# calderpg/fast_kinematic_simulator

Measured on AMD Instinct MI355X. Metric: particle-microsteps/sec, 7-DOF arm vs 256³ SDF, at 1/2/4/8 MI355X, higher is better.
Workload: dtype f64

## Files before the change

### fast_kinematic_simulator_amd/_capi.py

```python
from __future__ import annotations

import ctypes
import os
from ctypes import POINTER, c_char_p, c_double, c_float, c_int32, c_int64, c_uint8, c_uint32, c_uint64, c_void_p

LIB_NAME = "libfks_hip.so"
LIB_PATH = os.environ.get("FKS_LIB_PATH") or os.path.join(os.path.dirname(os.path.abspath(__file__)), LIB_NAME)

FKS_OK = 0
STATUS_NAMES = {
    0: "FKS_OK",
    1: "FKS_ERR_INVALID_ARGUMENT",
    2: "FKS_ERR_HIP",
    3: "FKS_ERR_NO_ROBOT",
    4: "FKS_ERR_OUT_OF_MEMORY",
    5: "FKS_ERR_UNSUPPORTED",
    6: "FKS_ERR_NO_DEVICE",
}

ROBOT_LINKED, ROBOT_SE2, ROBOT_SE3 = 0, 1, 2
JOINT_FIXED, JOINT_REVOLUTE, JOINT_CONTINUOUS, JOINT_PRISMATIC = 0, 1, 2, 4
KIN_LINK_TRANSFORMS, KIN_POINTS, KIN_APPLY_CONTROL_INPUT = 0, 1, 2
OK, ERR_INVALID_ARGUMENT, ERR_HIP, ERR_NO_ROBOT, ERR_OUT_OF_MEMORY, ERR_UNSUPPORTED, ERR_NO_DEVICE = 0, 1, 2, 3, 4, 5, 6

NUM_PHASES = 16
PHASE_NAMES = ["particle", "control", "step_setup", "micro_input", "micro_fk", "env_check", "self_check", "corrections",
               "solve", "resolve_apply", "output", "env_rounds_skipped", "env_rounds_evaluated", "corr_rounds_skipped",
               "corr_rounds_evaluated", "wave_residency"]
PHASE_COUNTS = {"env_rounds_skipped", "env_rounds_evaluated", "corr_rounds_skipped", "corr_rounds_evaluated", "wave_residency"}

PARTICLE_ERR_MICROSTEP_MOTION = 0x1
PARTICLE_ERR_NORMAL_OOB = 0x2
PARTICLE_ERR_ZERO_DIRECTION = 0x4
PARTICLE_ERR_RNG_EXHAUSTED = 0x8
PARTICLE_ERR_SELF_CAPACITY = 0x10
PARTICLE_ERR_KEY_RANGE = 0x20
PARTICLE_ERR_MICROSTEP_CAP = 0x40
PARTICLE_ERR_SELF_SINGULAR = 0x80
PARTICLE_ERR_NO_NOISE_BIN = 0x100


class SolverParams(ctypes.Structure):
    _fields_ = [
        ("forward_simulation_time", c_double),
        ("simulation_shortcut_distance", c_double),
        ("environment_collision_check_tolerance", c_double),
        ("resolve_correction_step_scaling_decay_rate", c_double),
        ("resolve_correction_initial_step_size", c_double),
        ("resolve_correction_min_step_scaling", c_double),
        ("max_resolver_iterations", c_uint32),
        ("resolve_correction_step_scaling_decay_iterations", c_uint32),
        ("failed_resolves_end_motion", c_uint32),
        ("reserved", c_uint32),
    ]


class GridGeometry(ctypes.Structure):
    _fields_ = [("origin", c_double * 12), ("resolution", c_double), ("num_cells", c_int64 * 3)]


class Environment(ctypes.Structure):
    _fields_ = [
        ("collision_map", GridGeometry),
        ("sdf", GridGeometry),
        ("sdf_values", POINTER(c_float)),
        ("sdf_oob_value", c_float),
        ("reserved", c_uint32),
        ("normals", GridGeometry),
        ("normal_offsets", POINTER(c_uint32)),
        ("normal_entries", POINTER(c_double)),
    ]


class DofController(ctypes.Structure):
    _fields_ = [
        ("kp", c_double),
        ("ki", c_double),
        ("kd", c_double),
        ("integral_clamp", c_double),
        ("velocity_limit", c_double),
        ("acceleration_limit", c_double),
        ("max_sensor_noise", c_double),
        ("max_actuator_proportional_noise", c_double),
        ("max_actuator_minimum_noise", c_double),
    ]


class JointDesc(ctypes.Structure):
    _fields_ = [
        ("parent_link", c_int32),
        ("child_link", c_int32),
        ("type", c_int32),
        ("reserved", c_int32),
        ("origin", c_double * 12),
        ("axis", c_double * 3),
        ("limit_lower", c_double),
        ("limit_upper", c_double),
    ]


class SampledActuator(ctypes.Structure):
    _fields_ = [
        ("num_bins", c_uint32),
        ("bin_elements", c_uint32),
        ("bin_bounds", POINTER(c_double)),
        ("bin_samples", POINTER(c_double)),
    ]


class RobotDesc(ctypes.Structure):
    _fields_ = [
        ("robot_type", c_int32),
# ... 354 lines not shown
```

### fast_kinematic_simulator_amd/csrc/fks_kernels.hip

```cpp
#if !defined(__HIPCC_RTC__)
#include <hip/hip_runtime.h>
#include <stdint.h>
#endif

#include "fks_capi.h"
#include "fks_control.h"
#include "fks_device.h"
#include "fks_portable_math.h"
#include "fks_se3.h"

namespace fksd {

using fks_math::clamp;
using fks_math::dabs;
using fks_math::dmax;
using fks_math::dmin;
using fks_math::dsqrt;

#if defined(FKS_SHAPE_L)
struct RobotShape {
    int L, J, D, W, G;
};
constexpr RobotShape kShape{FKS_SHAPE_L, FKS_SHAPE_J, FKS_SHAPE_D, FKS_SHAPE_W, FKS_SHAPE_G};
constexpr LdsLayout kShapeLayout = make_lds_layout(FKS_SHAPE_L, FKS_SHAPE_J, FKS_SHAPE_D, FKS_SHAPE_W, FKS_SHAPE_G,
// ... 233 lines not shown
        c[3] = lo0;
        k0 += W0;
        k1 += W1;
    }
}
__device__ __forceinline__ double u53(uint32_t a, uint32_t b) {
    const uint64_t bits = (((uint64_t)a << 32) | (uint64_t)b) >> 11;
    return (double)bits * (1.0 / 9007199254740992.0);
}
__device__ double tn_sample(uint32_t k0, uint32_t k1, uint64_t particle, uint32_t step, uint32_t micro, uint32_t dof,
                            uint32_t* err) {
    const double mean = 0.0, stddev = 0.5, lo = -2.0, hi = 2.0;
    uint32_t attempt = 0;
    while (attempt < 64u) {
        double x, y, r2;
        for (;;) {
            uint32_t c[4] = {(uint32_t)particle, step, micro,
                             ((uint32_t)(particle >> 32) << 16) | ((dof & 0xffu) << 8) | attempt};
            philox4x32_10(c, k0, k1);
            x = 2.0 * u53(c[0], c[1]) - 1.0;
            y = 2.0 * u53(c[2], c[3]) - 1.0;
            r2 = x * x + y * y;
            if (!(r2 > 1.0 || r2 == 0.0)) break;
            if (++attempt >= 64u) {
                *err |= FKS_PARTICLE_ERR_RNG_EXHAUSTED;
                return 0.0;
            }
        }
        const double mult = dsqrt(-2.0 * fks_math::log(r2) / r2);
        const double n1 = (y * mult) * 1.0 + 0.0;
        const double n2 = (x * mult) * 1.0 + 0.0;
        if ((n1 <= hi) && (n1 >= lo)) return mean + stddev * n1;
        if ((n2 <= hi) && (n2 >= lo)) return mean + stddev * n2;
        ++attempt;
    }
    *err |= FKS_PARTICLE_ERR_RNG_EXHAUSTED;
    return 0.0;
}

__device__ double sampled_pick(uint32_t k0, uint32_t k1, uint64_t particle, uint32_t step, uint32_t micro, uint32_t dof,
                               uint32_t elems) {
    uint32_t c[4] = {(uint32_t)particle, step, micro, ((uint32_t)(particle >> 32) << 16) | ((dof & 0xffu) << 8)};
    philox4x32_10(c, k0, k1);
    uint32_t pick = (uint32_t)(u53(c[0], c[1]) * (double)elems);
    if (pick >= elems) pick = elems - 1u;
    return (double)pick;
}

struct Sim;
__device__ FKS_SHAPE_INLINE void refill_noise(Sim& s, uint32_t micro0, uint32_t M);
__device__ __forceinline__ double noise_sample(Sim& s, uint32_t micro);

__device__ __forceinline__ bool grid_index(const GridDev& g, const D4& p, int32_t idx[3]) {
    const D4 q = xform4(g.inv, p);
    const double v[3] = {q.x * g.inv_res, q.y * g.inv_res, q.z * g.inv_res};
    bool ok = true;
#pragma unroll
    for (int a = 0; a < 3; ++a) {
        const bool fin = (v[a] > -2147483648.0) && (v[a] < 2147483647.0);
        idx[a] = fin ? (int32_t)v[a] : -1;
        ok = ok && fin && idx[a] >= 0 && (int64_t)idx[a] < g.n[a];
    }
    return ok;
}
__device__ __forceinline__ uint32_t grid_brick(const GridDev& g, int32_t i, int32_t j, int32_t k) {
    return brick_cell(g.nb, (uint32_t)i, (uint32_t)j, (uint32_t)k);
}

#ifndef FKS_ASM_LANE
#if defined(FKS_SHAPE_LEAN) && FKS_SHAPE_LEAN
#define FKS_ASM_LANE 1
#else
#define FKS_ASM_LANE 0
#endif
#endif
#if defined(FKS_SHAPE_TYPE) && FKS_SHAPE_TYPE == 0
#define FKS_PID_REGS 0
#else
#define FKS_PID_REGS 1
#endif
#ifndef FKS_PAR_PROOF
#define FKS_PAR_PROOF 1
#endif
#ifndef FKS_NO_SKIP_PROOFS
#define FKS_NO_SKIP_PROOFS 0
#endif
extern __shared__ __attribute__((aligned(16))) double fks_lds[];

struct Sim {
    const SimArgs* A;
    double* lds_block;
    double* scratch;
    int lane_v;
    __device__ __forceinline__ int lane() const {
#if FKS_ASM_LANE
        int ln;
        asm volatile("v_mbcnt_lo_u32_b32 %0, -1, 0\n\tv_mbcnt_hi_u32_b32 %0, -1, %0" : "=v"(ln));
        return ln;
#else
        return lane_v;
#endif
    }
    uint32_t step;
    uint32_t err;
    uint64_t lane_bytes;
    uint64_t local;
    uint32_t micro_count, resolver_count, step_count, lsq_rows;
    __device__ __forceinline__ double* lds() const { return lds_block; }
    __device__ __forceinline__ double* shared() const { return fks_lds; }
    __device__ __forceinline__ uint64_t pid() const { return A->first_pid + local; }
    __device__ __forceinline__ uint32_t* stats() const { return reinterpret_cast<uint32_t*>(lds() + LAY(*A).misc + 24); }
    __device__ __forceinline__ uint64_t* phase() const { return reinterpret_cast<uint64_t*>(lds() + LAY(*A).misc + 8); }
    __device__ __forceinline__ uint64_t* totals() const { return reinterpret_cast<uint64_t*>(lds() + LAY(*A).misc + 32); }
    __device__ __forceinline__ const JointDev* joints() const { return reinterpret_cast<const JointDev*>(shared() + LAY(*A).joints); }
    __device__ __forceinline__ const fks_dof_controller* ctrl() const {
        return reinterpret_cast<const fks_dof_controller*>(shared() + LAY(*A).ctrl);
    }
    __device__ __forceinline__ const int32_t* dofj() const { return reinterpret_cast<const int32_t*>(shared() + LAY(*A).dofj); }
    __device__ __forceinline__ const double* base() const { return shared() + LAY(*A).base; }
    __device__ __forceinline__ double* pid_state() const { return scratch + SLAY(*A).pid; }
#if FKS_PID_REGS
    double pid_integral, pid_last;
#endif
    double* rstate;
    double* selfref;
    bool self_nonempty;
    bool tcur_valid;
    uint32_t tr_steps, tr_cfgs;
};
template <int RT>
__device__ __forceinline__ void pid_get(const Sim& s, int ln, double* integral, double* last) {
    if constexpr (RT == FKS_ROBOT_LINKED) {
        *integral = s.pid_state()[ln];
        *last = s.pid_state()[kWave + ln];
    } else {
#if FKS_PID_REGS
        *integral = s.pid_integral;
        *last = s.pid_last;
#endif
    }
}
template <int RT>
__device__ __forceinline__ void pid_set(Sim& s, int ln, double integral, double last) {
    if constexpr (RT == FKS_ROBOT_LINKED) {
        s.pid_state()[ln] = integral;
        s.pid_state()[kWave + ln] = last;
    } else {
#if FKS_PID_REGS
        s.pid_integral = integral;
        s.pid_last = last;
#endif
    }
}
enum { kTotSteps = 0, kTotMicro, kTotResolver, kTotLsq, kTotErrors, kWaveTotals };

__device__ __forceinline__ int opaque_lane(int ln) {
    asm volatile("" : "+v"(ln));
    return ln;
}

__device__ __forceinline__ uint64_t* self_counters(const Sim& s) { return reinterpret_cast<uint64_t*>(s.lds() + LAY(*s.A).misc + 28); }

template <bool TR>
__device__ __forceinline__ void trace_config(Sim& s, const double* cfg, uint32_t micro, uint32_t kind) {
    if constexpr (TR) {
        const SimArgs& A = *s.A;
        const uint32_t k = s.tr_cfgs++;
        if (k < A.tr_cfg_cap) {
            const uint64_t rec = s.local * (uint64_t)A.tr_cfg_cap + k;
            if (s.lane() < RDIM(A.R, W)) A.tr_cfg[rec * (uint64_t)RDIM(A.R, W) + s.lane()] = cfg[s.lane()];
            if (s.lane() == 0) {
                A.tr_tags[3 * rec] = s.step;
                A.tr_tags[3 * rec + 1] = micro;
                A.tr_tags[3 * rec + 2] = kind;
            }
        }
    }
}
template <bool TR>
__device__ __forceinline__ void trace_step(Sim& s, const double* u, const double* ustep, uint32_t M) {
    if constexpr (TR) {
        const SimArgs& A = *s.A;
        const uint32_t k = s.tr_steps++;
        if (k < A.tr_step_cap) {
            const int D = RDIM(A.R, D);
            const uint64_t rec = s.local * (uint64_t)A.tr_step_cap + k;
            if (s.lane() < D) {
                A.tr_inputs[rec * 2ull * (uint64_t)D + s.lane()] = u[s.lane()];
                A.tr_inputs[rec * 2ull * (uint64_t)D + D + s.lane()] = ustep[s.lane()];
            }
            if (s.lane() == 0) A.tr_micro[rec] = M;
        }
    }
}

#ifndef FKS_PHASE_TIMERS
#define FKS_PHASE_TIMERS 0
#endif
__device__ __forceinline__ uint64_t tick() {
    if constexpr (FKS_PHASE_TIMERS) return __builtin_amdgcn_s_memtime();
    return 0;
}
__device__ __forceinline__ void tock(Sim& s, int phase, uint64_t t0) {
    if constexpr (FKS_PHASE_TIMERS)
        if (s.lane() == 0) s.phase()[phase] += tick() - t0;
}
__device__ __forceinline__ void count_event(Sim& s, int slot, uint64_t n) {
    if constexpr (FKS_PHASE_TIMERS)
        if (s.lane() == 0) s.phase()[slot] += n;
}

__device__ __noinline__ void refill_noise_lanes(const SimArgs* __restrict__ Ap, double* lds, int ln, uint64_t pid, uint32_t step,
                                                uint32_t micro0, uint32_t M) {
    const SimArgs& A = *Ap;
    const int D = RDIM(A.R, D);
    const int per = kWave / D;
    double* nz = lds + LAY(A).noise;
    uint32_t* ne = reinterpret_cast<uint32_t*>(lds + LAY(A).noise_err);
    if (ln < per * D) {
        const uint32_t m = micro0 + (uint32_t)(ln / D);
        if (m < M) {
            uint32_t e = 0;
            const uint32_t dof = (uint32_t)(ln % D);
            if ((A.R.sampled_mask >> dof) & 1ull)
                nz[ln] = sampled_pick(A.key0, A.key1, pid, step, m, dof, load_sampled(A.R.sampled, (int)dof).elems);
            else
                nz[ln] = tn_sample(A.key0, A.key1, pid, step, m, dof, &e);
            ne[ln] = e;
        }
    }
    wsync();
}
__device__ FKS_SHAPE_INLINE void refill_noise(Sim& s, uint32_t micro0, uint32_t M) {
    refill_noise_lanes(s.A, s.lds(), s.lane(), s.pid(), s.step, micro0, M);
}
__device__ __forceinline__ double noise_sample(Sim& s, uint32_t micro) {
    const SimArgs& A = *s.A;
    const int D = RDIM(A.R, D);
    const int slot = (int)(micro % (uint32_t)(kWave / D)) * D + s.lane();
    s.err |= reinterpret_cast<const uint32_t*>(s.lds() + LAY(A).noise_err)[slot];
    return s.lds()[LAY(A).noise + slot];
}

__device__ double estimate_distance(const SimArgs& A, const D4& p, bool* inb, uint64_t* bytes) {
    int32_t idx[3];
    if (!grid_index(A.sdf_g, p, idx)) {
        *inb = false;
        return (double)A.oob;
    }
    *inb = true;
    *bytes += 28;
    const GridDev& g = A.sdf_g;
    double grad[3];
#pragma unroll
    for (int a = 0; a < 3; ++a) {
        int32_t lo[3] = {idx[0], idx[1], idx[2]}, hi[3] = {idx[0], idx[1], idx[2]};
        lo[a] = (idx[a] - 1 > 0) ? idx[a] - 1 : 0;
        hi[a] = ((int64_t)idx[a] + 1 < g.n[a] - 1) ? idx[a] + 1 : (int32_t)(g.n[a] - 1);
        const double inv = g.inv_res_span[hi[a] - lo[a]];
        const float diff = gp(A.sdf)[grid_brick(g, hi[0], hi[1], hi[2])] - gp(A.sdf)[grid_brick(g, lo[0], lo[1], lo[2])];
        grad[a] = (double)diff * inv;
    }
    const D3 c = xform3(g.org, D3{g.res * ((double)idx[0] + 0.5), g.res * ((double)idx[1] + 0.5), g.res * ((double)idx[2] + 0.5)});
    const double dx = p.x - c.x, dy = p.y - c.y, dz = p.z - c.z;
    const double nominal = (double)gp(A.sdf)[grid_brick(g, idx[0], idx[1], idx[2])];
    const double corrected = (nominal >= 0.0) ? nominal - (g.res * 0.5) : nominal + (g.res * 0.5);
    const double adjustment = (dx * grad[0] + dy * grad[1]) + dz * grad[2];
    const double estimate = corrected + adjustment;
    if ((corrected >= 0.0) == (estimate >= 0.0)) return estimate;
    if (corrected >= 0.0) return g.res * 0.0625;
    return g.res * -0.0625;
}

__device__ bool lookup_normal(const SimArgs& A, const D4& loc, const D4& dir, D3* out, uint32_t* err, uint64_t* bytes) {
    *out = D3{0.0, 0.0, 0.0};
    int32_t idx[3];
    if (!A.has_normals || !grid_index(A.nrm_g, loc, idx)) return false;
    const uint64_t range = gp(reinterpret_cast<const uint64_t*>(A.nrange))[grid_brick(A.nrm_g, idx[0], idx[1], idx[2])];
    const uint32_t begin = (uint32_t)range, end = (uint32_t)(range >> 32);
    *bytes += 4;
    if (begin == end) return true;
    *bytes += 56ull * (uint64_t)(end - begin);
    const double direction_norm = dsqrt(sqnorm4(dir));
    if (!(direction_norm > 0.0)) {
        *err |= FKS_PARTICLE_ERR_ZERO_DIRECTION;
        return true;
    }
    const double ux = dir.x / direction_norm, uy = dir.y / direction_norm, uz = dir.z / direction_norm;
    const FKS_GLOBAL double* e0 = gp(A.nent) + 6ull * begin;
    const double n0 = e0[3], n1 = e0[4], n2 = e0[5];
    int64_t best = -1;
    double best_dot = -__builtin_huge_val();
// ... 2255 lines not shown
            perm[transp[k]] = t;
        }
    }
    wsync();
    if (nz == 0) return;
    for (int k = 0; k < nz; ++k) {
        const double tau = hco[k];
        const double* ck = col(k);
        if (Rn - (uint32_t)k == 1u) {
            wsync();
            if (ln == 0) c[k] = c[k] * (1.0 - tau);
            wsync();
        } else if (tau != 0.0) {
            double acc = 0.0;
            for (uint32_t r = (uint32_t)ln; r < Rn; r += kWave)
                if (r > (uint32_t)k) acc = acc + ck[r] * c[r];
            double tmp = bfly_sum(acc);
            tmp = tmp + c[k];
            wsync();
            if (ln == 0) c[k] = c[k] - tau * tmp;
            for (uint32_t r = (uint32_t)ln; r < Rn; r += kWave)
                if (r > (uint32_t)k) c[r] = c[r] - (tau * ck[r]) * tmp;
            wsync();
        }
    }
    for (int ii = nz - 1; ii >= 0; --ii) {
        const double ci = c[ii];
        if (ci != 0.0) {
            const double* cc = col(ii);
            const double v = ci / cc[ii];
            wsync();
            if (ln == 0) c[ii] = v;
            if (ln < ii) c[ln] = c[ln] - v * cc[ln];
            wsync();
        }
    }
    if (ln < nz) x[perm[ln]] = c[ln];
    wsync();
}

__device__ __noinline__ void individual_jacobians_solve(Sim& s, uint32_t Rn, double* x) {
    const int ln = s.lane();
    const int D = RDIM(s.A->R, D);
    double* acc = s.lds() + LAY(*s.A).real;
    for (uint32_t r0 = 0; r0 < Rn; r0 += 3u) {
        if (D < kWave)
            qr_solve_cols<8>(s.A, s.lds(), s.scratch, ln, 3u, x, r0);
        else
            qr_solve(s.A, s.lds(), s.scratch, ln, 3u, x, r0);
        if (ln < D) acc[ln] = (r0 == 0u) ? x[ln] : acc[ln] + x[ln];
        wsync();
    }
    if (ln < D) x[ln] = (Rn == 0u) ? 0.0 : acc[ln];
    wsync();
}

template <int RT, bool TR, bool IND, int COOP = 0>
__device__ FKS_SHAPE_INLINE int resolve_step(Sim& s, const double* particle_cfg, double* res_cfg, bool allow_contacts, bool* out_collided,
                            bool* out_failed, double*& Tcur, double*& Tprev) {
    const SimArgs& A = *s.A;
    const RobotDev& R = A.R;
    const int ln = s.lane();
    const int W = RDIM(R, W), D = RDIM(R, D);
    double* u = s.lds() + LAY(*s.A).u;
    double* ustep = s.lds() + LAY(*s.A).ustep;
    double* cfg_tmp = s.lds() + LAY(*s.A).cfg_tmp;
    double* cfg_prev = s.lds() + LAY(*s.A).cfg_prev;
    double* cfg_act = s.lds() + LAY(*s.A).cfg_act;
    double* x = s.lds() + LAY(*s.A).x;
    double* real = s.lds() + LAY(*s.A).real;
    double* Ttmp;
    {
        double* b0 = s.lds() + LAY(*s.A).Tcur;
        double* b1 = s.lds() + LAY(*s.A).Tprev;
        double* b2 = s.lds() + LAY(*s.A).Ttmp;
        Ttmp = (b0 != Tcur && b0 != Tprev) ? b0 : ((b1 != Tcur && b1 != Tprev) ? b1 : b2);
    }
    double* cfg = s.lds() + LAY(*s.A).cfg_work;
    *out_collided = false;
    *out_failed = false;
    uint64_t t0 = tick();
    if (ln < W) cfg[ln] = particle_cfg[ln];
    wsync();
    if (!s.tcur_valid) fk<RT>(s, cfg, Tcur);
    apply_input<RT>(s, cfg, u, cfg_tmp, false, 0);
    fk<RT>(s, cfg_tmp, Ttmp);
    s.tcur_valid = false;
    const double computed_step_motion = max_point_motion(s, Tcur, Ttmp);
    const double raw_steps = __builtin_ceil(computed_step_motion / A.target_micro);
    if (!(raw_steps <= 1048576.0)) {
        s.err |= FKS_PARTICLE_ERR_MICROSTEP_CAP;
        return 1;
    }
    uint32_t M = (uint32_t)raw_steps;
    if (M < 1u) M = 1u;
    if (ln < D) ustep[ln] = u[ln] / (double)M;
    wsync();
    bool proven = false;
    {
        const double term = (ln < D) ? dabs(ustep[ln]) * gp(R.dof_lever)[ln] : 0.0;
        const double bound = bfly_sum(0.0 + term);
        proven = !FKS_NO_SKIP_PROOFS && bound * (1.0 + 1e-6) + 1e-12 < A.allowed_micro;
    }
    if (!proven) {
        apply_input<RT>(s, cfg, ustep, cfg_tmp, false, 0);
        fk<RT>(s, cfg_tmp, Ttmp);
        const double micro_motion = max_point_motion(s, Tcur, Ttmp);
        if (micro_motion > A.allowed_micro) {
            s.err |= FKS_PARTICLE_ERR_MICROSTEP_MOTION;
            return 1;
        }
    }
    tock(s, FKS_PHASE_STEP_SETUP, t0);
    trace_step<TR>(s, u, ustep, M);
    bool collided = false;
    const uint32_t noise_per = (uint32_t)(kWave / RDIM(R, D));
    bool pair_ready = false;
    uint32_t pair_err = 0;
    for (uint32_t micro = 0; micro < M; ++micro) {
        s.lane_v = opaque_lane(s.lane_v);
        const int ln = s.lane();
        s.micro_count++;
        if (ln < W) cfg_prev[ln] = cfg[ln];
        wsync();
        t0 = tick();
        const bool predicted = pair_ready;
        if (predicted) {
            if (ln < W) cfg[ln] = cfg_tmp[ln];
            s.err |= pair_err;
            wsync();
        } else {
            if (micro % (uint32_t)(kWave / RDIM(R, D)) == 0u)
                refill_noise(s, micro, M);
            apply_input<RT>(s, cfg_prev, ustep, cfg, true, micro);
        }
        s.err = wave_or(s.err);
        tock(s, FKS_PHASE_MICRO_INPUT, t0);
        if (s.err) {
            if (ln < W) res_cfg[ln] = cfg_prev[ln];
            wsync();
            return 1;
        }
        t0 = tick();
        if (predicted) {
            double* t = Tprev;
            Tprev = Tcur;
            Tcur = Ttmp;
            Ttmp = t;
            pair_ready = false;
        } else {
            {
                double* t = Tprev;
                Tprev = Tcur;
                Tcur = t;
            }
            pair_ready = false;
            bool pair = false;
            if constexpr (RT == FKS_ROBOT_LINKED) {
                pair = LAY(A).fk_pair && micro + 1u < M && ((micro + 1u) % noise_per) != 0u;
                if (pair) {
                    const uint32_t err_keep = s.err;
                    apply_input<RT>(s, cfg, ustep, cfg_tmp, true, micro + 1u);
                    pair_err = s.err;
                    s.err = err_keep;
                    fk_pair(s, cfg, Tcur, cfg_tmp, Ttmp);
                    pair_ready = true;
                }
            }
            if (!pair)
                fk<RT>(s, cfg, Tcur);
        }
        tock(s, FKS_PHASE_MICRO_FK, t0);
        bool in_collision = check_collision<RT, COOP>(s, Tprev, Tcur, cfg);
        if (s.err) return 1;
        if (in_collision) pair_ready = false;
        trace_config<TR>(s, cfg, micro, FKS_TRACE_POST_ACTION);
        if (in_collision) collided = true;
        if (in_collision && allow_contacts) {
            if (ln < W) cfg_act[ln] = cfg[ln];
            wsync();
            uint32_t iters = 0;
            constexpr bool kScalingLds = RT == FKS_ROBOT_LINKED;
            double* scaling_p = s.lds() + LAY(*s.A).misc + 38;
            double scaling_reg = A.S.resolve_correction_initial_step_size;
            if (kScalingLds) {
                if (ln == 0) *scaling_p = scaling_reg;
                wsync();
            }
            while (in_collision) {
                s.lane_v = opaque_lane(s.lane_v);
                const int ln = s.lane();
                s.resolver_count++;
                t0 = tick();
                uint32_t Rn;
                if constexpr (COOP > 0)
                    Rn = collect_corrections_coop<RT, COOP>(s, Tprev, Tcur, cfg_act);
                else
                    Rn = collect_corrections<RT>(s, Tprev, Tcur, cfg_act);
                s.lsq_rows += Rn;
                s.err = wave_or(s.err);
                tock(s, FKS_PHASE_CORRECTIONS, t0);
// ... 447 lines not shown
}

__device__ __forceinline__ uint32_t job_of(const SimArgs* __restrict__ args, uint32_t g, int ln) {
    const uint32_t* __restrict__ first = args->job_first;
    uint32_t lo = 0, count = args->num_jobs + 1u;
    while (count > (uint32_t)kWave) {
        const uint32_t stride = (count + (uint32_t)kWave - 1u) / (uint32_t)kWave;
        const uint32_t at = (uint32_t)ln * stride;
        const bool le = at < count && first[lo + at] <= g;
        const uint32_t c = (uint32_t)__builtin_popcountll(__builtin_amdgcn_ballot_w64(le));
        const uint32_t rest = count - (c - 1u) * stride;
        lo += (c - 1u) * stride;
        count = rest < stride ? rest : stride;
    }
    const bool le = (uint32_t)ln < count && first[lo + (uint32_t)ln] <= g;
    const uint32_t c = (uint32_t)__builtin_popcountll(__builtin_amdgcn_ballot_w64(le));
    return (uint32_t)__builtin_amdgcn_readfirstlane((int)(lo + c - 1u));
}

template <int RT, bool TR, bool IND = false, bool LEAN = false, int COOP = 0, bool PATH = false, bool JOBS = false>
__device__ __forceinline__ void simulate_particles(const SimArgs* __restrict__ args, double* lds_mem) {
    const SimArgs& A = *args;
    auto batch_n = [&]() -> uint64_t {
        if constexpr (JOBS)
            return args->jobs_total;
        else
            return A.n;
    };
    const RobotDev& R = A.R;
    const int wave = __builtin_amdgcn_readfirstlane((int)(threadIdx.x >> 6));
    double* shared = lds_mem;
    {
        const int t = (int)threadIdx.x, nt = (int)blockDim.x;
        uint64_t* dj = reinterpret_cast<uint64_t*>(shared + LAY(A).joints);
        const uint64_t* sj = reinterpret_cast<const uint64_t*>(R.joints);
        for (int k = t; k < RDIM(R, J) * kJointWords; k += nt) dj[k] = sj[k];
        uint64_t* dc = reinterpret_cast<uint64_t*>(shared + LAY(A).ctrl);
        const uint64_t* sc = reinterpret_cast<const uint64_t*>(R.ctrl);
        for (int k = t; k < RDIM(R, D) * kCtrlWords; k += nt) dc[k] = sc[k];
        int32_t* dd = reinterpret_cast<int32_t*>(shared + LAY(A).dofj);
        if (RT == FKS_ROBOT_LINKED && t < RDIM(R, D)) dd[t] = gp(R.dof_joint)[t];
        if (t < 12) shared[LAY(A).base + t] = R.base[t];
        if (RT == FKS_ROBOT_LINKED) {
            for (int k = t; k < 8 * RDIM(R, G); k += nt)
                shared[LAY(A).gbox + k] = (k % 8 == 7) ? (double)gp(R.geom_link)[k / 8] : gp(R.geom_box)[7 * (k / 8) + k % 8];
            uint32_t* lp = reinterpret_cast<uint32_t*>(shared + LAY(A).gpairs);
            for (int k = t; k < RDIM(R, npairs) && k < kLdsPairs; k += nt)
                lp[k] = (uint32_t)gp(R.pairs)[2 * k] | ((uint32_t)gp(R.pairs)[2 * k + 1] << 16);
        }
        if (t < RDIM(R, nrounds) && t < kWave) {
            const RoundDev rd = load_round(R.rounds, t);
            shared[LAY(A).rounds + 2 * t] = (double)rd.link;
            shared[LAY(A).rounds + 2 * t + 1] = rd.radius;
        }
        __syncthreads();
    }
    if constexpr (COOP > 0) {
        if (wave != 0) {
            coop_helper<RT, COOP>(args, lds_mem, wave);
            return;
        }
    }
    Sim s;
    s.A = args;
    s.lds_block = lds_mem + LAY(A).shared_total + (uint64_t)wave * LAY(A).total;
    s.scratch = A.scratch + ((uint64_t)blockIdx.x * (COOP > 0 ? 1u : (blockDim.x >> 6)) + (uint64_t)wave) * A.scratch_per_wave;
    s.lane_v = lane_id();
    s.rstate = LEAN ? s.scratch + SLAY(A).rstate : s.lds() + LAY(A).rstate;
    s.selfref = LEAN ? s.scratch + SLAY(A).selfref : s.lds() + LAY(A).selfref;
    if (s.lane() < RDIM(R, nrounds)) s.rstate[kRoundState * s.lane() + 12] = kInvalidRound;
    wsync();
    const int ln = s.lane();
    const int W = RDIM(R, W), D = RDIM(R, D);
    double* cfg = s.lds() + LAY(*s.A).cfg;
    double* res_cfg = s.lds() + LAY(*s.A).cfg_res;
    double* u = s.lds() + LAY(*s.A).u;
    unsigned long long* next_particle = reinterpret_cast<unsigned long long*>(s.lds() + LAY(*s.A).misc + 31);
    uint32_t* seg_seen = reinterpret_cast<uint32_t*>(s.lds() + LAY(*s.A).misc + 30);
    const uint32_t nseg = A.nseg;
    const uint32_t nsegs = (PATH && JOBS) ? nseg * A.path_legs_max : (PATH ? nseg * A.path_legs : nseg);
    uint64_t carry = kNoTicket;
    bool carry_heavy = false;
    if (ln < 8) s.stats()[ln] = 0;
    if (ln < FKS_NUM_PHASES) s.phase()[ln] = 0;
    if (ln < kWaveTotals) s.totals()[ln] = 0;
    s.lane_bytes = 0;
    if (ln < 2) self_counters(s)[ln] = 0;
    if (ln == 0) *reinterpret_cast<uint64_t*>(s.lds() + LAY(*s.A).misc + 6) = 0;
    if (ln == 0) s.phase()[FKS_PHASE_WAVE_RESIDENCY] = 0ull - __builtin_amdgcn_s_memrealtime();
    wsync();
    while (true) {
        uint64_t ticket;
        uint32_t prio = 0;
        if (carry != kNoTicket) {
            ticket = carry;
            carry = kNoTicket;
            prio = carry_heavy ? 2u : (A.seg_heavy_prio > 1u ? 1u : 0u);
        } else {
            if (ln == 0) {
                const uint64_t t = __hip_atomic_fetch_add(A.queue, 1ull, __ATOMIC_RELAXED, __HIP_MEMORY_SCOPE_AGENT);
                const uint64_t sg = (batch_n() > 0) ? t / batch_n() : (uint64_t)nsegs;
                uint32_t run = 1;
                if (sg > 0 && sg < (uint64_t)nsegs) {
                    uint32_t* done = A.seg_done + (t - sg * batch_n());
                    uint32_t v = __hip_atomic_load(done, __ATOMIC_RELAXED, __HIP_MEMORY_SCOPE_AGENT);
                    run = (v == (uint32_t)sg &&
                           __hip_atomic_compare_exchange_strong(done, &v, (uint32_t)sg | kSegClaimed, __ATOMIC_RELAXED,
                                                                __ATOMIC_RELAXED, __HIP_MEMORY_SCOPE_AGENT))
                              ? 1u
                              : 0u;
                }
                *next_particle = t;
                *seg_seen = run;
            }
            wsync();
            ticket = *next_particle;
            const uint32_t run = *seg_seen;
            wsync();
            if ((batch_n() > 0 ? ticket / batch_n() : (uint64_t)nsegs) >= (uint64_t)nsegs) {
                const uint64_t bytes = wave_sum_u64(s.lane_bytes);
                if (ln == 0) {
                    s.phase()[FKS_PHASE_WAVE_RESIDENCY] += __builtin_amdgcn_s_memrealtime();
                    for (int k = 0; k < 8; ++k)
                        if (s.stats()[k]) atomicAdd(A.counters + k, (unsigned long long)s.stats()[k]);
                    const uint64_t* wt = s.totals();
                    if (wt[kTotSteps]) atomicAdd(A.counters + kCntSteps, (unsigned long long)wt[kTotSteps]);
                    if (wt[kTotMicro]) atomicAdd(A.counters + kCntMicrosteps, (unsigned long long)wt[kTotMicro]);
                    if (wt[kTotResolver]) atomicAdd(A.counters + kCntResolver, (unsigned long long)wt[kTotResolver]);
                    if (wt[kTotLsq]) atomicAdd(A.counters + kCntLsqRows, (unsigned long long)wt[kTotLsq]);
                    if (bytes) atomicAdd(A.counters + kCntSdfBytes, (unsigned long long)bytes);
                    if (wt[kTotErrors]) atomicAdd(A.counters + kCntErrorParticles, (unsigned long long)wt[kTotErrors]);
                    const uint64_t* sc = self_counters(s);
                    if (sc[0]) atomicAdd(A.counters + kCntSelfChecks, (unsigned long long)sc[0]);
                    if (sc[1]) atomicAdd(A.counters + kCntSelfPoints, (unsigned long long)sc[1]);
                    for (int k = 0; k < FKS_NUM_PHASES; ++k)
                        if (s.phase()[k]) atomicAdd(A.counters + kPhaseBase + k, (unsigned long long)s.phase()[k]);
                }
                if constexpr (COOP > 0) {
                    if (ln == 0) coop_box(s)->cmd = kCoopExit;
                    coop_sync();
                }
                break;
            }
            if (!run) continue;
            claim_fence();
        }
        if (A.seg_heavy_prio) {
            if (prio == 2u)
                __builtin_amdgcn_s_setprio(2);
            else if (prio == 1u)
                __builtin_amdgcn_s_setprio(1);
            else
                __builtin_amdgcn_s_setprio(0);
        }
        uint64_t seg = ticket / batch_n();
        const uint64_t global = ticket - seg * batch_n();
        uint32_t leg = 0;
        if constexpr (PATH) {
            leg = (uint32_t)__builtin_amdgcn_readfirstlane((int)((uint32_t)seg / nseg));
            seg -= (uint64_t)leg * nseg;
        }
        uint32_t rec = leg;
        if constexpr (JOBS) rec = job_of(args, (uint32_t)global, ln);
        if constexpr (PATH && JOBS) {
            rec = (uint32_t)__builtin_amdgcn_readfirstlane((int)args->job_first[args->num_jobs + 1u + rec]);
            if (leg >= args[rec].path_legs) continue;
            rec += leg;
        }
        const SimArgs& A = (PATH || JOBS) ? args[rec] : *args;
        if constexpr (PATH || JOBS) s.A = &A;
        const uint64_t local = JOBS ? global - A.job_base : global;
        const uint32_t step_begin = (uint32_t)seg * A.seg_steps;
        const uint32_t step_end = (seg + 1 == (uint64_t)nseg) ? A.T : step_begin + A.seg_steps;
        double* st = A.seg_state + local * (uint64_t)A.seg_stride;
        s.local = local;
        s.tr_steps = 0;
        s.tr_cfgs = 0;
        s.err = 0;
        s.micro_count = 0;
        s.resolver_count = 0;
        s.lsq_rows = 0;
        s.step_count = 0;
        if (ln == 0) s.phase()[FKS_PHASE_PARTICLE] -= __builtin_amdgcn_s_memtime();
        s.self_nonempty = false;
        s.tcur_valid = false;
        if (ln == 0) s.selfref[RDIM(R, D)] = -1.0;
        const double* start = A.starts + local * (uint64_t)W;
        auto start_at = [&](int i) -> double {
            if constexpr (PATH) {
                if (leg > 0) return load_coherent(start + i);
            }
            return start[i];
        };
        const double* target = (A.num_targets == A.n) ? A.targets + local * (uint64_t)W : A.targets;
        bool collided = false;
        bool any_failed = false;
        if (seg == 0) {
            if (ln < D)
                pid_set<RT>(s, ln, A.pid_io ? A.pid_io[local * 2ull * (uint64_t)D + ln] : 0.0,
                            A.pid_io ? A.pid_io[local * 2ull * (uint64_t)D + D + ln] : 0.0);
            if constexpr (RT == FKS_ROBOT_LINKED) {
                if (ln < D) {
                    const JointDev& jd = s.joints()[s.dofj()[ln]];
                    cfg[ln] = (jd.type == FKS_JOINT_CONTINUOUS) ? fks_math::wrap_revolute(start_at(ln))
                                                                : clamp(start_at(ln), jd.lo, jd.hi);
                }
            } else if constexpr (RT == FKS_ROBOT_SE2) {
                if (ln < 3) cfg[ln] = (ln == 2) ? fks_math::wrap_revolute(start_at(2)) : start_at(ln);
            } else {
                if (ln < 12) cfg[ln] = start_at(ln);
            }
            if constexpr (PATH) {
                if (leg > 0 && ln < RDIM(R, nrounds)) s.rstate[kRoundState * ln + 12] = kInvalidRound;
            }
        } else {
            if (ln < W) cfg[ln] = load_coherent(A.out_q + local * (uint64_t)W + ln);
            if (ln < D) pid_set<RT>(s, ln, load_coherent(st + ln), load_coherent(st + D + ln));
            const uint64_t* sw = reinterpret_cast<const uint64_t*>(st + 2 * D);
            const uint64_t flags = load_coherent_u64(sw);
// ... 402 lines not shown
```

### include/fks_capi.h

```cpp
#ifndef FKS_CAPI_H
#define FKS_CAPI_H

#if defined(__HIPCC_RTC__)
using __hip_internal::int16_t;
using __hip_internal::int32_t;
using __hip_internal::int64_t;
using __hip_internal::int8_t;
using __hip_internal::uint16_t;
using __hip_internal::uint32_t;
using __hip_internal::uint64_t;
using __hip_internal::uint8_t;
#ifndef INT32_MIN
#define INT32_MIN (-2147483647 - 1)
#endif
#else
#include <stdint.h>
#endif

#ifdef __cplusplus
extern "C" {
#endif

#define FKS_ABI_VERSION 10

// ... 196 lines not shown
    uint32_t* out_resolver_iterations;
    uint32_t* out_error_flags;
} fks_job;
#define FKS_MAX_JOBS 65536u
fks_status fks_forward_simulate_jobs(fks_context* ctx, const fks_job* jobs, uint64_t num_jobs);
fks_status fks_forward_simulate_jobs_device(fks_context* ctx, const fks_job* jobs, uint64_t num_jobs, void* stream,
                                            int32_t synchronize);

typedef struct {
    const double* starts;
    uint64_t n;
    const double* waypoints;
    uint64_t num_legs;
    uint64_t num_targets;
    uint64_t first_particle_id;
    int32_t allow_contacts;
    int32_t reserved;
    double* out_positions;
    uint8_t* out_collided;
    uint32_t* out_microsteps;
    uint32_t* out_resolver_iterations;
    uint32_t* out_error_flags;
} fks_path_job;
#define FKS_MAX_PATH_JOB_LEGS FKS_MAX_JOBS
fks_status fks_forward_simulate_path_jobs(fks_context* ctx, const fks_path_job* jobs, uint64_t num_jobs);
fks_status fks_forward_simulate_path_jobs_device(fks_context* ctx, const fks_path_job* jobs, uint64_t num_jobs, void* stream,
                                                 int32_t synchronize);

fks_status fks_check_config_collision(fks_context* ctx, const double* configs, uint64_t n,
                                      double inflation_ratio, uint8_t* out_collided,
                                      uint32_t* out_error_flags);
fks_status fks_check_config_collision_device(fks_context* ctx, const double* d_configs, uint64_t n,
                                             double inflation_ratio, uint8_t* d_out_collided,
                                             uint32_t* d_out_error_flags, void* stream,
                                             int32_t synchronize);
fks_status fks_get_last_check_counters(const fks_context* ctx, fks_call_counters* out);

#define FKS_TRACE_POST_ACTION 0u
#define FKS_TRACE_RESOLVER_STEP 1u
#define FKS_TRACE_RESOLVE_FAILED 2u
#define FKS_TRACE_CONTACT_STOP 3u
typedef struct {
    uint32_t step_capacity;
    uint32_t config_capacity;
    double* step_inputs;
    uint32_t* step_microsteps;
    double* configs;
    uint32_t* config_tags;
    uint32_t* num_steps;
    uint32_t* num_configs;
} fks_trace;

fks_status fks_forward_simulate_traced(fks_context* ctx, const double* starts, uint64_t n,
                                       const double* targets, uint64_t num_targets,
                                       int32_t allow_contacts, double* out_positions,
                                       uint8_t* out_collided, uint32_t* out_microsteps,
                                       uint32_t* out_resolver_iterations, uint32_t* out_error_flags,
                                       const fks_trace* trace);

fks_status fks_forward_simulate_traced_mutable(fks_context* ctx, const double* starts, uint64_t n, const double* targets,
                                               uint64_t num_targets, int32_t allow_contacts, double* controller_state,
                                               double* out_positions, uint8_t* out_collided, uint32_t* out_microsteps,
                                               uint32_t* out_resolver_iterations, uint32_t* out_error_flags,
                                               const fks_trace* trace);

#define FKS_KIN_LINK_TRANSFORMS 0
#define FKS_KIN_POINTS 1
#define FKS_KIN_APPLY_CONTROL_INPUT 2
fks_status fks_kinematics(fks_context* ctx, int32_t mode, const double* configs, uint64_t n, const double* inputs,
                          double* out);
fks_status fks_robot_sizes(const fks_context* ctx, int32_t* num_links, int32_t* num_points, int32_t* num_dofs,
                           int32_t* config_width);

fks_status fks_set_call_index(fks_context* ctx, uint64_t call_index);
uint64_t fks_get_call_index(const fks_context* ctx);

fks_status fks_get_statistics(const fks_context* ctx, fks_statistics* out);
fks_status fks_reset_statistics(fks_context* ctx);
fks_status fks_set_statistics(fks_context* ctx, const fks_statistics* stats);
fks_status fks_reset_generators(fks_context* ctx, uint64_t prng_seed);
int32_t fks_get_debug_level(const fks_context* ctx);
int32_t fks_set_debug_level(fks_context* ctx, int32_t debug_level);
fks_status fks_get_last_call_counters(const fks_context* ctx, fks_call_counters* out);
#define FKS_NUM_PHASES 16
enum fks_phase {
    FKS_PHASE_PARTICLE = 0,
    FKS_PHASE_CONTROL = 1,
    FKS_PHASE_STEP_SETUP = 2,
    FKS_PHASE_MICRO_INPUT = 3,
    FKS_PHASE_MICRO_FK = 4,
    FKS_PHASE_ENV_CHECK = 5,
    FKS_PHASE_SELF_CHECK = 6,
    FKS_PHASE_CORRECTIONS = 7,
    FKS_PHASE_SOLVE = 8,
    FKS_PHASE_RESOLVE_APPLY = 9,
    FKS_PHASE_OUTPUT = 10,
    FKS_PHASE_ENV_ROUNDS_SKIPPED = 11,
    FKS_PHASE_ENV_ROUNDS_EVALUATED = 12,
    FKS_PHASE_CORR_ROUNDS_SKIPPED = 13,
    FKS_PHASE_CORR_ROUNDS_EVALUATED = 14,
    FKS_PHASE_WAVE_RESIDENCY = 15
};
fks_status fks_get_phase_cycles(const fks_context* ctx, int which, uint64_t* out );
fks_status fks_get_launch_geometry(const fks_context* ctx, uint32_t* resident_waves, uint64_t* lds_bytes_per_group);
typedef enum {
    FKS_KERNEL_NONE = 0,
    FKS_KERNEL_THROUGHPUT = 1,
    FKS_KERNEL_SMALL_BATCH = 2,
    FKS_KERNEL_SHAPED = 3,
    FKS_KERNEL_TRACED = 4,
    FKS_KERNEL_INDIVIDUAL = 5,
    FKS_KERNEL_COOPERATIVE = 6,
    FKS_KERNEL_SHAPED_SMALL_BATCH = 7,
    FKS_KERNEL_PATH = 8,
    FKS_KERNEL_PATH_SMALL_BATCH = 9,
    FKS_KERNEL_JOBS = 10,
    FKS_KERNEL_JOBS_SMALL_BATCH = 11,
    FKS_KERNEL_PATH_JOBS = 12,
    FKS_KERNEL_PATH_JOBS_SMALL_BATCH = 13
} fks_kernel_kind;
typedef struct fks_launch_info {
    uint32_t resident_waves;
    uint32_t waves_per_group;
    uint64_t lds_bytes_per_group;
    uint32_t small_batch_resident_waves;
    uint32_t standard_layout_resident_waves;
    int32_t fk_pair;
    int32_t lean;
    int32_t last_kernel;
    int32_t last_check_kernel;
    uint32_t cooperative_resident_particles;
    uint32_t cooperative_waves_per_particle;
} fks_launch_info;
fks_status fks_get_launch_info(const fks_context* ctx, fks_launch_info* out);
fks_status fks_set_segment_steps(fks_context* ctx, uint32_t controller_steps);
fks_status fks_set_segment_policy(fks_context* ctx, uint32_t heavy_resolver_per_step, uint32_t heavy_priority);
fks_status fks_set_segment_heavy_relative(fks_context* ctx, uint32_t times_mean);
fks_status fks_set_small_batch_kernel(fks_context* ctx, int32_t enabled);
fks_status fks_set_cooperative_waves(fks_context* ctx, int32_t enabled);
fks_status fks_set_individual_jacobians(fks_context* ctx, int32_t simulate_with_individual_jacobians);
typedef enum {
    FKS_SPECIALIZE_OFF = 0,
    FKS_SPECIALIZE_ON = 1,
    FKS_SPECIALIZE_NO_PROOFS = 2
} fks_specialization_mode;
fks_status fks_set_specialization(fks_context* ctx, int32_t mode);
typedef struct fks_specialization_info {
    int32_t enabled;
    int32_t active;
    int32_t from_cache;
    int32_t pending;
    double compile_seconds;
    uint64_t launches;
    char shape[64];
    int32_t failed;
    int32_t reserved;
    char message[512];
} fks_specialization_info;
fks_status fks_get_specialization(const fks_context* ctx, fks_specialization_info* out);

fks_status fks_get_total_counters(const fks_context* ctx, fks_call_counters* out);
fks_status fks_reset_total_counters(fks_context* ctx);
fks_status fks_set_total_counters(fks_context* ctx, const fks_call_counters* totals);

fks_status fks_robot_control_action(const fks_robot_desc* robot, const double* config, const double* target,
                                    double controller_interval, double* pid_state, double* out_control);
fks_status fks_robot_apply_control_input(const fks_robot_desc* robot, const double* config, const double* input,
                                         const double* unit_noise, double* out_config);

typedef struct {
    double pose[12];
    double extents[3];
    uint32_t object_id;
    uint32_t reserved;
} fks_obstacle;

typedef struct fks_env_handle fks_env_handle;

fks_status fks_env_build(const fks_obstacle* obstacles, int32_t num_obstacles,
                         double resolution, const double* grid_origin,
                         const int64_t* num_cells, fks_env_handle** out);
typedef struct {
    uint64_t cells;
    uint64_t obstacle_samples;
// ... 66 lines not shown
```

Measured before the change: 303.4 million.

## Skip step-setup FK via single-microstep proof and pair speculative first microstep

In shaped kernels, step setup first tries a lever-arm bound on the full input. When the bound proves one microstep suffices, the forward-kinematics trial passes are skipped entirely. Otherwise, for linked robots with fk_pair, it guesses the microstep count from the previous step, precomputes the first microstep's configuration, and runs FK for the full-step trial and the first microstep together. If the guess matches, the paired result seeds the microstep loop. This adds three phase counters and extra branching, and a wrong guess wastes the speculative input application and noise refill.

```diff
diff --git a/fast_kinematic_simulator_amd/_capi.py b/fast_kinematic_simulator_amd/_capi.py
--- a/fast_kinematic_simulator_amd/_capi.py
+++ b/fast_kinematic_simulator_amd/_capi.py
@@ -23,11 +23,12 @@
 KIN_LINK_TRANSFORMS, KIN_POINTS, KIN_APPLY_CONTROL_INPUT = 0, 1, 2
 OK, ERR_INVALID_ARGUMENT, ERR_HIP, ERR_NO_ROBOT, ERR_OUT_OF_MEMORY, ERR_UNSUPPORTED, ERR_NO_DEVICE = 0, 1, 2, 3, 4, 5, 6
 
-NUM_PHASES = 16
+NUM_PHASES = 19
 PHASE_NAMES = ["particle", "control", "step_setup", "micro_input", "micro_fk", "env_check", "self_check", "corrections",
                "solve", "resolve_apply", "output", "env_rounds_skipped", "env_rounds_evaluated", "corr_rounds_skipped",
-               "corr_rounds_evaluated", "wave_residency"]
-PHASE_COUNTS = {"env_rounds_skipped", "env_rounds_evaluated", "corr_rounds_skipped", "corr_rounds_evaluated", "wave_residency"}
+               "corr_rounds_evaluated", "wave_residency", "setup_proven_single", "setup_pairs_used", "setup_pairs_discarded"]
+PHASE_COUNTS = {"env_rounds_skipped", "env_rounds_evaluated", "corr_rounds_skipped", "corr_rounds_evaluated", "wave_residency",
+                "setup_proven_single", "setup_pairs_used", "setup_pairs_discarded"}
 
 PARTICLE_ERR_MICROSTEP_MOTION = 0x1
 PARTICLE_ERR_NORMAL_OOB = 0x2
diff --git a/fast_kinematic_simulator_amd/csrc/fks_kernels.hip b/fast_kinematic_simulator_amd/csrc/fks_kernels.hip
--- a/fast_kinematic_simulator_amd/csrc/fks_kernels.hip
+++ b/fast_kinematic_simulator_amd/csrc/fks_kernels.hip
@@ -339,6 +339,17 @@
 #ifndef FKS_PAR_PROOF
 #define FKS_PAR_PROOF 1
 #endif
+#if defined(FKS_SHAPE_TYPE)
+#define FKS_SETUP_DEFAULT 1
+#else
+#define FKS_SETUP_DEFAULT 0
+#endif
+#ifndef FKS_SETUP_PROOF
+#define FKS_SETUP_PROOF FKS_SETUP_DEFAULT
+#endif
+#ifndef FKS_SETUP_PAIR
+#define FKS_SETUP_PAIR FKS_SETUP_DEFAULT
+#endif
 #ifndef FKS_NO_SKIP_PROOFS
 #define FKS_NO_SKIP_PROOFS 0
 #endif
@@ -462,9 +473,19 @@
     if constexpr (FKS_PHASE_TIMERS)
         if (s.lane() == 0) s.phase()[phase] += tick() - t0;
 }
+constexpr int kPhaseLdsSlots = 16;
+static_assert(FKS_NUM_PHASES - kPhaseLdsSlots <= 7, "sixteen spare int words, two in use");
+__device__ __forceinline__ uint64_t* phase_extra(const Sim& s) {
+    return reinterpret_cast<uint64_t*>(reinterpret_cast<int32_t*>(s.lds() + LAY(*s.A).ints) + 2 * kMaxDofs) + 1;
+}
 __device__ __forceinline__ void count_event(Sim& s, int slot, uint64_t n) {
     if constexpr (FKS_PHASE_TIMERS)
-        if (s.lane() == 0) s.phase()[slot] += n;
+        if (s.lane() == 0) {
+            if (slot < kPhaseLdsSlots)
+                s.phase()[slot] += n;
+            else
+                phase_extra(s)[slot - kPhaseLdsSlots] += n;
+        }
 }
 
 __device__ __noinline__ void refill_noise_lanes(const SimArgs* __restrict__ Ap, double* lds, int ln, uint64_t pid, uint32_t step,
@@ -2886,6 +2907,86 @@
     uint64_t t0 = tick();
     if (ln < W) cfg[ln] = particle_cfg[ln];
     wsync();
+#if FKS_SETUP_PROOF || FKS_SETUP_PAIR
+    [[maybe_unused]] const bool had_prev = s.tcur_valid;
+    if (!s.tcur_valid) fk<RT>(s, cfg, Tcur);
+    constexpr bool kSetupPair = FKS_SETUP_PAIR && RT == FKS_ROBOT_LINKED;
+    [[maybe_unused]] uint32_t* m_prev = reinterpret_cast<uint32_t*>(s.lds() + LAY(*s.A).misc + 37);
+    const bool pair_setup = kSetupPair && LAY(A).fk_pair;
+    double* cfg_trial = pair_setup ? cfg_act : cfg_tmp;
+    double* Ttrial = pair_setup ? Tprev : Ttmp;
+    bool setup_hit = false;
+    uint32_t setup_err = 0;
+    bool single = false;
+    if (FKS_SETUP_PROOF && !FKS_NO_SKIP_PROOFS) {
+        const double term = (ln < D) ? dabs(u[ln]) * gp(R.dof_lever)[ln] : 0.0;
+        const double bound = bfly_sum(0.0 + term) * (1.0 + 1e-6) + 1e-12;
+        single = bound < A.target_micro && bound < A.allowed_micro;
+    }
+    uint32_t M = 1u;
+    if (single) {
+        s.tcur_valid = false;
+        if (ln < D) ustep[ln] = u[ln];
+        wsync();
+        count_event(s, FKS_PHASE_SETUP_PROVEN, 1);
+    } else {
+        uint32_t Mg = 0;
+        if constexpr (kSetupPair) {
+            if (pair_setup && had_prev) Mg = (uint32_t)__builtin_amdgcn_readfirstlane((int)*m_prev);
+        }
+        if (Mg) {
+            if constexpr (kSetupPair) {
+                if (ln < D) ustep[ln] = u[ln] / (double)Mg;
+                wsync();
+                refill_noise(s, 0u, Mg);
+                apply_input<RT>(s, cfg, u, cfg_trial, false, 0);
+                const uint32_t err_keep = s.err;
+                apply_input<RT>(s, cfg, ustep, cfg_tmp, true, 0u);
+                setup_err = s.err;
+                s.err = err_keep;
+                fk_pair(s, cfg_trial, Ttrial, cfg_tmp, Ttmp);
+            }
+        } else {
+            apply_input<RT>(s, cfg, u, cfg_trial, false, 0);
+            fk<RT>(s, cfg_trial, Ttrial);
+        }
+        s.tcur_valid = false;
+        const double computed_step_motion = max_point_motion(s, Tcur, Ttrial);
+        const double raw_steps = __builtin_ceil(computed_step_motion / A.target_micro);
+        if (!(raw_steps <= 1048576.0)) {
+            s.err |= FKS_PARTICLE_ERR_MICROSTEP_CAP;
+            return 1;
+        }
+        M = (uint32_t)raw_steps;
+        if (M < 1u) M = 1u;
+        if (ln < D) ustep[ln] = u[ln] / (double)M;
+        wsync();
+        bool proven = false;
+        {
+            const double term = (ln < D) ? dabs(ustep[ln]) * gp(R.dof_lever)[ln] : 0.0;
+            const double bound = bfly_sum(0.0 + term);
+            proven = !FKS_NO_SKIP_PROOFS && bound * (1.0 + 1e-6) + 1e-12 < A.allowed_micro;
+        }
+        if (!proven) {
+            apply_input<RT>(s, cfg, ustep, cfg_trial, false, 0);
+            fk<RT>(s, cfg_trial, Ttrial);
+            const double micro_motion = max_point_motion(s, Tcur, Ttrial);
+            if (micro_motion > A.allowed_micro) {
+                s.err |= FKS_PARTICLE_ERR_MICROSTEP_MOTION;
+                return 1;
+            }
+        }
+        if (Mg) {
+            setup_hit = M == Mg;
+            count_event(s, setup_hit ? FKS_PHASE_SETUP_PAIR_USED : FKS_PHASE_SETUP_PAIR_DROPPED, 1);
+        }
+    }
+    if constexpr (kSetupPair) {
+        if (pair_setup) {
+            if (ln == 0) *m_prev = M;
+        }
+    }
+#else
     if (!s.tcur_valid) fk<RT>(s, cfg, Tcur);
     apply_input<RT>(s, cfg, u, cfg_tmp, false, 0);
     fk<RT>(s, cfg_tmp, Ttmp);
@@ -2915,12 +3016,15 @@
             return 1;
         }
     }
+    const bool setup_hit = false;
+    const uint32_t setup_err = 0;
+#endif
     tock(s, FKS_PHASE_STEP_SETUP, t0);
     trace_step<TR>(s, u, ustep, M);
     bool collided = false;
     const uint32_t noise_per = (uint32_t)(kWave / RDIM(R, D));
-    bool pair_ready = false;
-    uint32_t pair_err = 0;
+    bool pair_ready = setup_hit;
+    uint32_t pair_err = setup_err;
     for (uint32_t micro = 0; micro < M; ++micro) {
         s.lane_v = opaque_lane(s.lane_v);
         const int ln = s.lane();
@@ -3534,7 +3638,9 @@
     uint64_t carry = kNoTicket;
     bool carry_heavy = false;
     if (ln < 8) s.stats()[ln] = 0;
-    if (ln < FKS_NUM_PHASES) s.phase()[ln] = 0;
+    if (ln < kPhaseLdsSlots) s.phase()[ln] = 0;
+    if constexpr (FKS_PHASE_TIMERS)
+        if (ln < FKS_NUM_PHASES - kPhaseLdsSlots) phase_extra(s)[ln] = 0;
     if (ln < kWaveTotals) s.totals()[ln] = 0;
     s.lane_bytes = 0;
     if (ln < 2) self_counters(s)[ln] = 0;
@@ -3585,8 +3691,12 @@
                     const uint64_t* sc = self_counters(s);
                     if (sc[0]) atomicAdd(A.counters + kCntSelfChecks, (unsigned long long)sc[0]);
                     if (sc[1]) atomicAdd(A.counters + kCntSelfPoints, (unsigned long long)sc[1]);
-                    for (int k = 0; k < FKS_NUM_PHASES; ++k)
+                    for (int k = 0; k < kPhaseLdsSlots; ++k)
                         if (s.phase()[k]) atomicAdd(A.counters + kPhaseBase + k, (unsigned long long)s.phase()[k]);
+                    if constexpr (FKS_PHASE_TIMERS)
+                        for (int k = kPhaseLdsSlots; k < FKS_NUM_PHASES; ++k)
+                            if (phase_extra(s)[k - kPhaseLdsSlots])
+                                atomicAdd(A.counters + kPhaseBase + k, (unsigned long long)phase_extra(s)[k - kPhaseLdsSlots]);
                 }
                 if constexpr (COOP > 0) {
                     if (ln == 0) coop_box(s)->cmd = kCoopExit;
diff --git a/include/fks_capi.h b/include/fks_capi.h
--- a/include/fks_capi.h
+++ b/include/fks_capi.h
@@ -302,7 +302,7 @@
 int32_t fks_get_debug_level(const fks_context* ctx);
 int32_t fks_set_debug_level(fks_context* ctx, int32_t debug_level);
 fks_status fks_get_last_call_counters(const fks_context* ctx, fks_call_counters* out);
-#define FKS_NUM_PHASES 16
+#define FKS_NUM_PHASES 19
 enum fks_phase {
     FKS_PHASE_PARTICLE = 0,
     FKS_PHASE_CONTROL = 1,
@@ -319,7 +319,10 @@
     FKS_PHASE_ENV_ROUNDS_EVALUATED = 12,
     FKS_PHASE_CORR_ROUNDS_SKIPPED = 13,
     FKS_PHASE_CORR_ROUNDS_EVALUATED = 14,
-    FKS_PHASE_WAVE_RESIDENCY = 15
+    FKS_PHASE_WAVE_RESIDENCY = 15,
+    FKS_PHASE_SETUP_PROVEN = 16,
+    FKS_PHASE_SETUP_PAIR_USED = 17,
+    FKS_PHASE_SETUP_PAIR_DROPPED = 18
 };
 fks_status fks_get_phase_cycles(const fks_context* ctx, int which, uint64_t* out );
 fks_status fks_get_launch_geometry(const fks_context* ctx, uint32_t* resident_waves, uint64_t* lds_bytes_per_group);
```

New measurement: 302.1 million, median of 2. No clear change (-0.5%).
